# themattinthehatt/behavenet

Measured on AMD Instinct MI355X. Metric: AE training frames/sec (128x128x1, batch 256), higher is better.
Workload: dtype f32; 1 GPU; configs[1]: conv AE default arch, 1x128x128 f32 frames resident in HBM, 12 latents, batch 256 (chunks 200+56), fwd+bwd+Adam(amsgrad)

## Files before the change

behavenet_amd/_hip.py:

```python

import ctypes
import os

import torch

_LIB_NAME = 'libbehavenet_hip.so'
_LIB_PATH = os.environ.get('BN_HIP_LIB') or os.path.join(
    os.path.dirname(os.path.abspath(__file__)), _LIB_NAME)
_lib = None

ACT_NONE, ACT_LRELU, ACT_SIGMOID = 0, 1, 2

PROF_NONE, PROF_CONV_FWD, PROF_CONV_BWD_D, PROF_CONV_BWD_W = 0, 1, 2, 3
PROF_CONVT_FWD, PROF_CONVT_BWD_D, PROF_CONVT_BWD_W, PROF_ADAM = 4, 5, 6, 7
PROF_LINEAR_FWD, PROF_LINEAR_BWD = 8, 9

_c_int, _c_float, _c_size_t, _c_void_p = ctypes.c_int, ctypes.c_float, ctypes.c_size_t, ctypes.c_void_p

_CONV_GEOM = [_c_int] * 12
_ACT_WS = [_c_int, _c_float, _c_void_p, _c_size_t, _c_void_p]

OP_CONV_FWD, OP_CONV_BWD_D, OP_CONV_BWD_W = 1, 2, 3
OP_CONVT_FWD, OP_CONVT_BWD_D, OP_CONVT_BWD_W = 4, 5, 6

SIGNATURES = {
    'bn_version': (_c_int, []),
    'bn_build_arch': (ctypes.c_char_p, []),
    'bn_error_string': (ctypes.c_char_p, [_c_int]),
    'bn_set_force_generic': (_c_int, [_c_int]),
    'bn_set_bigk1_block_bytes': (_c_size_t, [_c_size_t]),
    'bn_conv_ws_bytes': (_c_size_t, [_c_int] + _CONV_GEOM),
    'bn_conv_taps_bytes': (_c_size_t, [_c_int] + _CONV_GEOM),
    'bn_conv_taps_pad': (_c_int, [_c_int, _c_void_p, _c_void_p, _c_void_p, _c_void_p]),
    'bn_conv_taps_hint': (_c_int, [_c_void_p, _c_void_p]),
    'bn_conv2d_fwd': (_c_int, [_c_void_p] * 4 + _CONV_GEOM + _ACT_WS),
    'bn_conv2d_fwd_u8_ws_bytes': (_c_size_t, _CONV_GEOM + [_c_int]),
    'bn_conv2d_fwd_u8': (_c_int, [_c_void_p] * 4 + _CONV_GEOM + _ACT_WS),
    'bn_conv2d_bwd_data': (_c_int, [_c_void_p] * 4 + _CONV_GEOM + _ACT_WS),
    'bn_conv2d_bwd_weight': (
        _c_int, [_c_void_p] * 4 + _CONV_GEOM + [_c_int, _c_void_p, _c_size_t, _c_void_p]),
    'bn_convT2d_fwd': (_c_int, [_c_void_p] * 4 + _CONV_GEOM + _ACT_WS),
    'bn_convT2d_bwd_data': (_c_int, [_c_void_p] * 4 + _CONV_GEOM + _ACT_WS),
    'bn_convT2d_bwd_weight': (
        _c_int, [_c_void_p] * 4 + _CONV_GEOM + [_c_int, _c_void_p, _c_size_t, _c_void_p]),
    'bn_batchnorm_ws_bytes': (_c_size_t, [_c_int, _c_int]),
    'bn_batchnorm_stats': (_c_int, [_c_void_p] * 3 + [_c_int] * 3 + [_c_void_p, _c_size_t, _c_void_p]),
    'bn_batchnorm_finalize': (_c_int, [_c_void_p] * 5 + [_c_int] + [_c_float] * 3 + [_c_void_p]),
    'bn_batchnorm_act_fwd': (_c_int, [_c_void_p] * 6 + [_c_int] * 4 + [_c_float, _c_void_p]),
    'bn_batchnorm_train_fwd_chunks': (
        _c_int, [_c_void_p] * 11 + [_c_int] * 3 + [_c_float, _c_int, _c_float, _c_void_p, _c_size_t,
                                                  _c_void_p]),
    'bn_batchnorm_act_bwd_chunks': (
        _c_int, [_c_void_p] * 10 + [_c_int, _c_void_p] + [_c_int] * 4 + [_c_float, _c_void_p, _c_size_t,
                                                                        _c_void_p]),
    'bn_batchnorm_act_bwd': (
        _c_int, [_c_void_p] * 9 + [_c_int] * 6 + [_c_float, _c_void_p, _c_size_t, _c_void_p]),
    'bn_batchnorm_moment': (_c_int, [_c_void_p] * 3 + [_c_int] * 3 + [_c_void_p, _c_size_t, _c_void_p]),
    'bn_batchnorm_bwd_reduce': (
        _c_int, [_c_void_p] * 7 + [_c_int] * 4 + [_c_float, _c_void_p, _c_size_t, _c_void_p]),
    'bn_batchnorm_bwd_apply': (
        _c_int, [_c_void_p] * 9 + [_c_int] * 3 + [_c_float, _c_int, _c_float, _c_void_p]),
    'bn_maxpool2d_fwd': (_c_int, [_c_void_p] * 3 + [_c_int] * 9 + [_c_void_p]),
    'bn_maxpool2d_bwd': (_c_int, [_c_void_p] * 3 + [_c_int] * 9 + [_c_void_p]),
    'bn_maxpool2d_act_fwd': (_c_int, [_c_void_p] * 3 + [_c_int] * 4 + [ctypes.c_float, _c_void_p]),
    'bn_conv2d_pool2_act_fwd': (_c_int, [_c_void_p] * 5 + _CONV_GEOM + [_c_int, _c_float, _c_void_p]),
    'bn_conv2d_pool2_act_ok': (_c_int, _CONV_GEOM),
    'bn_conv2d_pool2_bwd_weight_ws_bytes': (_c_size_t, _CONV_GEOM),
    'bn_conv2d_pool2_bwd_weight': (
        _c_int, [_c_void_p] * 6 + _CONV_GEOM + [_c_int, _c_float, _c_int, _c_void_p, _c_size_t, _c_void_p]),
    'bn_maxpool2d_act_bwd': (_c_int, [_c_void_p] * 4 + [_c_int] * 4 + [ctypes.c_float, _c_void_p]),
    'bn_maxunpool2d_fwd': (_c_int, [_c_void_p] * 3 + [_c_int] * 3 + [_c_void_p]),
    'bn_maxunpool2d_fwd_k2': (_c_int, [_c_void_p] * 3 + [_c_int] * 3 + [_c_void_p]),
    'bn_maxunpool2d_bwd': (_c_int, [_c_void_p] * 3 + [_c_int] * 3 + [_c_void_p]),
    'bn_act_fwd': (_c_int, [_c_void_p] * 2 + [_c_size_t, _c_int, _c_float, _c_void_p]),
    'bn_act_bwd': (_c_int, [_c_void_p] * 3 + [_c_size_t, _c_int, _c_float, _c_void_p]),
    'bn_linear_ws_bytes': (_c_size_t, [_c_int] * 3),
    'bn_linear_fwd': (_c_int, [_c_void_p] * 4 + [_c_int] * 3 + [_c_void_p, _c_size_t, _c_void_p]),
# ... 194 lines not shown
        _ptr(x, 'x'), _ptr(dy, 'dy'), _ptr(dw, 'dw'), _ptr(db, 'db', allow_none=True), *geom,
        int(accumulate), ws, nb, _stream()), 'bn_conv2d_bwd_weight')


def convT2d_fwd(x, w, b, geom, act, slope, w5=None):
    N, Ci, Hi, Wi, Co, R, S, st, ct, cl, Ho, Wo = geom
    y = torch.empty((N, Co, Ho, Wo), dtype=torch.float32, device=x.device)
    ws, nb = _workspace(OP_CONVT_FWD, geom, x.device)
    _taps_hint(w, w5)
    _check(load().bn_convT2d_fwd(
        _ptr(x, 'x'), _ptr(w, 'w'), _ptr(b, 'b', allow_none=True), _ptr(y, 'y'), *geom,
        act, slope, ws, nb, _stream()), 'bn_convT2d_fwd')
    return y


def convT2d_bwd_data(dy, w, geom, dact_src, dact, slope, w5=None):
    N, Ci, Hi, Wi = geom[:4]
    dx = torch.empty((N, Ci, Hi, Wi), dtype=torch.float32, device=dy.device)
    ws, nb = _workspace(OP_CONVT_BWD_D, geom, dy.device)
    _taps_hint(w, w5)
    _check(load().bn_convT2d_bwd_data(
        _ptr(dy, 'dy'), _ptr(w, 'w'), _ptr(dx, 'dx'), _ptr(dact_src, 'dact_src', allow_none=True),
        *geom, dact, slope, ws, nb, _stream()), 'bn_convT2d_bwd_data')
    return dx


def convT2d_bwd_weight(x, dy, dw, db, geom, accumulate):
    ws, nb = _workspace(OP_CONVT_BWD_W, geom, x.device)
    _check(lib_call('bn_convT2d_bwd_weight')(
        _ptr(x, 'x'), _ptr(dy, 'dy'), _ptr(dw, 'dw'), _ptr(db, 'db', allow_none=True), *geom,
        int(accumulate), ws, nb, _stream()), 'bn_convT2d_bwd_weight')


def set_force_generic(on):
    global _generic_epoch
    _generic_epoch += 1
    return bool(load().bn_set_force_generic(1 if on else 0))


def set_bigk1_block_bytes(nbytes):
    return int(load().bn_set_bigk1_block_bytes(int(nbytes)))


def lib_call(name):
    return getattr(load(), name)


def _bn_ws(n, c, device):
    nbytes = load().bn_batchnorm_ws_bytes(n, c)
    return _arena(device, nbytes, 'bn'), nbytes


def batchnorm_train_fwd(x, gamma, beta, running_mean, running_var, momentum, eps, act, slope, y=None):
    n, c = x.shape[0], x.shape[1]
    hw = x.numel() // (n * c)
    mean = torch.empty((c,), dtype=torch.float32, device=x.device)
    var = torch.empty_like(mean)
    invstd = torch.empty_like(mean)
    ws, nb = _bn_ws(n, c, x.device)
    _check(load().bn_batchnorm_stats(_ptr(x, 'x'), _ptr(mean, 'mean'), _ptr(var, 'var'), n, c, hw,
                                     ws, nb, _stream()), 'bn_batchnorm_stats')
    cnt = n * hw
    unbias = cnt / (cnt - 1.0) if cnt > 1 else 1.0
    _check(load().bn_batchnorm_finalize(
        _ptr(mean, 'mean'), _ptr(var, 'var'), _ptr(invstd, 'invstd'),
        _ptr(running_mean, 'running_mean', allow_none=True),
# ... 500 lines not shown
```

behavenet_amd/csrc/bn_fast.h:

```cpp
#pragma once
#include "bn_common.h"

struct BnFastPlan {
    bool supported;
    const char* kernel_name;
    size_t ws_bytes;
    int variant;
    int a, b, c, d;
};

BnFastPlan bn_fast_down_plan(const BnGeom& g);
BnFastPlan bn_fast_up_plan(const BnGeom& g);
BnFastPlan bn_fast_wgrad_plan(const BnGeom& g);

int bn_launch_down_fast(const BnFastPlan& plan, const float* big, const float* w,
                        const float* bias, float* out, const float* dact_src, const BnGeom& g,
                        int act, int dact, float slope, void* ws, hipStream_t st);
int bn_launch_up_fast(const BnFastPlan& plan, const float* small, const float* w,
                      const float* bias, float* out, const float* dact_src, const BnGeom& g,
                      int act, int dact, float slope, void* ws, hipStream_t st);
int bn_launch_wgrad_fast(const BnFastPlan& plan, const float* small, const float* big, float* dw,
                         const BnGeom& g, int accumulate, void* ws, hipStream_t st,
                         float* db = nullptr, int bias_side = 0, bool* bias_done = nullptr);

// ... 14 lines not shown
int bn_launch_down2(int MR, int NR, const float* big, const float* w, const float* bias,
                    float* out, const float* dact_src, const BnGeom& g, int act, int dact,
                    float slope, hipStream_t st, int splits = 1, void* ws = nullptr);

BnFastPlan bn_wgrad4_plan(const BnGeom& g);
int bn_launch_wgrad4(const BnFastPlan& plan, const float* small, const float* big, float* dw,
                     const BnGeom& g, int accumulate, void* ws, hipStream_t st, float* db,
                     int bias_side, bool* bias_done);

BnFastPlan bn_s5_up_plan(const BnGeom& g);
BnFastPlan bn_s5_wgrad_plan(const BnGeom& g);
int bn_launch_up_s5(const float* small, const float* w, const float* bias, float* out,
                    const float* dact_src, const BnGeom& g, int act, int dact, float slope,
                    hipStream_t st);
int bn_launch_wgrad_s5(const float* small, const float* big, float* dw, const BnGeom& g,
                       int accumulate, hipStream_t st);

BnFastPlan bn_edge_wgrad_plan(const BnGeom& g);
int bn_launch_edge_wgrad(const BnFastPlan& plan, const float* small, const float* big, float* dw,
                         const BnGeom& g, int accumulate, void* ws, hipStream_t st,
                         float* db = nullptr, int bias_side = 0, bool* bias_done = nullptr);
bool bn_s1c1_ok(const BnGeom& g);
int bn_launch_s1c1(const float* big, const float* w, const float* bias, float* out, const float* dact_src,
                   const BnGeom& g, int act, int dact, float slope, hipStream_t st);
bool bn_s1in1_ok(const BnGeom& g);
int bn_launch_s1in1(const float* big, const float* w, const float* bias, float* out, const float* dact_src,
                    const BnGeom& g, int act, int dact, float slope, hipStream_t st);
BnFastPlan bn_edge_down_plan(const BnGeom& g);
const char* bn_edge_down_kernel_name(const BnGeom& g, int act, bool has_dact, bool u8);
const char* bn_edge_up_kernel_name(const BnGeom& g, bool loss);
int bn_launch_edge_down(const float* big, const float* w, const float* bias, float* out,
                        const float* dact_src, const BnGeom& g, int act, int dact, float slope,
                        hipStream_t st, const unsigned char* u8 = nullptr);
BnFastPlan bn_edge_up_plan(const BnGeom& g);
int bn_launch_edge_up(const float* small, const float* w, const float* bias, float* out,
                      const BnGeom& g, int act, float slope, hipStream_t st,
                      const float* target = nullptr, const float* mask = nullptr,
                      float* dpre = nullptr, float* partial = nullptr);
int bn_edge_up_parts_per_frame(const BnGeom& g);

bool bn_qgemm_supported(const BnGeom& g);
size_t bn_qgemm_ws_bytes(int role, const BnGeom& g);
int bn_launch_qgemm_down(const float* big, const float* w, const float* bias, float* out,
                         const float* dact_src, const BnGeom& g, int act, int dact, float slope,
                         void* ws, hipStream_t st);
int bn_launch_qgemm_up(const float* small, const float* w, const float* bias, float* out,
                       const float* dact_src, const BnGeom& g, int act, int dact, float slope,
                       void* ws, hipStream_t st);
int bn_launch_qgemm_wgrad(const float* small, const float* big, float* dw, const BnGeom& g,
                          int accumulate, void* ws, hipStream_t st);

bool bn_qg2_up_supported(const BnGeom& g, int act, int dact);
int bn_launch_qg2_up(const float* small, const float* w, const float* bias, float* out,
                     const float* dact_src, const BnGeom& g, int act, int dact, float slope,
                     hipStream_t st);
bool bn_qg2_wgrad_supported(const BnGeom& g);
int bn_launch_qg2_wgrad(const float* small, const float* big, float* dw, const BnGeom& g,
                        int accumulate, float* db, int bias_side, hipStream_t st);

bool bn_s5win_supported(const BnGeom& g);
size_t bn_s5win_ws_bytes(int role, const BnGeom& g);
int bn_launch_s5win_down(const float* big, const float* w, const float* bias, float* out,
                         const float* dact_src, const BnGeom& g, int act, int dact, float slope,
                         void* ws, hipStream_t st);
int bn_launch_s5win_up(const float* small, const float* w, const float* bias, float* out,
                       const float* dact_src, const BnGeom& g, int act, int dact, float slope,
// ... 8 lines not shown
```

behavenet_amd/csrc/capi.hip:

```cpp
#include <math.h>
#include <stdio.h>
#include <stdlib.h>
#include <string.h>
#include <hip/hip_ext.h>
#include "bn_common.h"
#include "bn_launch.h"
#include "bn_fast.h"

namespace {
struct ProfState {
    int family = BN_PROF_NONE;
    int C = 0, K = 0;
    static const int kMaxSlots = 2048;
    hipEvent_t ev[4 * kMaxSlots];
    bool taken[kMaxSlots], bracketed[kMaxSlots];
    int created = 0;
    int used = 0;
    double total_ms = 0.0, main_ms = 0.0;
    long launches = 0, main_launches = 0;
    bool bracket = true;
    int nth = -1, seen = 0;
    char kernel_name[96] = "";
} g_prof;

// ... 1261 lines not shown
}

extern "C" int bn_convT2d_bwd_data(const float* dy, const float* w, float* dx,
                                   const float* dact_src, int N, int Ci, int Hi, int Wi, int Co,
                                   int R, int S, int stride, int crop_t, int crop_l, int Ho,
                                   int Wo, int dact, float slope, void* ws, size_t ws_bytes,
                                   bn_stream_t stream) {
    TapsHintDrop hint_drop;
    if (!dy || !w || !dx) return BN_E_BADARG;
    const BnGeom g = convT_geom(N, Ci, Hi, Wi, Co, R, S, stride, crop_t, crop_l, Ho, Wo);
    if (!bn_geom_ok(g)) return BN_E_BADARG;
    return run_down(BN_PROF_CONVT_BWD_D, dy, w, nullptr, dx, dact_src, g, BN_ACT_NONE, dact, slope,
                    ws, ws_bytes, (hipStream_t)stream);
}

extern "C" int bn_convT2d_bwd_weight(const float* x, const float* dy, float* dw, float* db, int N,
                                     int Ci, int Hi, int Wi, int Co, int R, int S, int stride,
                                     int crop_t, int crop_l, int Ho, int Wo, int accumulate,
                                     void* ws, size_t ws_bytes, bn_stream_t stream) {
    TapsHintDrop hint_drop;
    if (!x || !dy || !dw) return BN_E_BADARG;
    const BnGeom g = convT_geom(N, Ci, Hi, Wi, Co, R, S, stride, crop_t, crop_l, Ho, Wo);
    if (!bn_geom_ok(g)) return BN_E_BADARG;
    hipStream_t st = (hipStream_t)stream;
    bool bias_done = false;
    int rc = run_wgrad(BN_PROF_CONVT_BWD_W, x, dy, dw, g, accumulate, ws, ws_bytes, st, db, 2,
                       &bias_done);
    if (rc) return rc;
    if (db && !bias_done)
        rc = bn_launch_channel_sum(dy, db, N, Co, Ho * Wo, accumulate, ws, ws_bytes, st);
    return rc;
}

extern "C" int bn_act_fwd(const float* x, float* y, size_t n, int act, float slope,
                          bn_stream_t stream) {
    if (!x || !y || n == 0) return BN_E_BADARG;
    return bn_launch_act_fwd(x, y, n, act, slope, (hipStream_t)stream);
}

extern "C" int bn_act_bwd(const float* dy, const float* y, float* dpre, size_t n, int act,
                          float slope, bn_stream_t stream) {
    if (!dy || !y || !dpre) return BN_E_BADARG;
    if (n == 0) return 0;
    return bn_launch_act_bwd(dy, y, dpre, n, act, slope, (hipStream_t)stream);
}

extern "C" size_t bn_batchnorm_ws_bytes(int N, int C) {
    return (N > 0 && C > 0) ? bn_batchnorm_ws_bytes_impl(N, C) : 0;
}

extern "C" int bn_batchnorm_stats(const float* x, float* mean, float* var, int N, int C, int HW,
                                  void* ws, size_t ws_bytes, bn_stream_t stream) {
    if (!x || !mean || !var || N <= 0 || C <= 0 || HW <= 0) return BN_E_BADARG;
    if (!ws || ws_bytes < bn_batchnorm_ws_bytes_impl(N, C)) return BN_E_WORKSPACE;
    return bn_launch_bn_stats(x, mean, var, N, C, HW, ws, (hipStream_t)stream);
}

extern "C" int bn_batchnorm_finalize(const float* mean, const float* var, float* invstd,
                                     float* running_mean, float* running_var, int C, float eps,
                                     float momentum, float unbias, bn_stream_t stream) {
    if (!mean || !var || !invstd || C <= 0) return BN_E_BADARG;
    return bn_launch_bn_finalize(mean, var, invstd, running_mean, running_var, C, eps, momentum,
                                 unbias, (hipStream_t)stream);
}

extern "C" int bn_batchnorm_act_fwd(const float* x, const float* mean, const float* invstd,
// ... 313 lines not shown
```

behavenet_amd/csrc/conv_edge.hip:

```cpp
#include <hip/hip_ext.h>
#include <stdlib.h>
#include "bn_common.h"
#include "bn_fast.h"
#include "bn_reduce.h"

typedef float floatx16 __attribute__((ext_vector_type(16)));

#define ED_THREADS 256
#define ED_OOB 0x7fffffff

__device__ __forceinline__ float ed_ld(__amdgpu_buffer_rsrc_t r, int byte_off) {
    return __builtin_bit_cast(float, __builtin_amdgcn_raw_buffer_load_b32(r, byte_off, 0, 0));
}

#define WC_ROWS 4
#define WC_W 64
#define WC_TPX (WC_ROWS * WC_W)
#define WC_SP (WC_TPX + 2)
#define WC_IH (2 * WC_ROWS + 3)
#define WC_RW (2 * WC_W + 4)
#define WC_KS (32 * WC_TPX / ED_THREADS)

#define WC_DECODE_GRID()                                                                    \
    int bch, bx, G;                                                                         \
// ... 1433 lines not shown
                : launch_down_c1s<BN_ACT_NONE, false, true, 4>(u8, w, bias, out, nullptr, g, slope, st, e0, e1);
        return act == BN_ACT_LRELU
            ? launch_down_c1s<BN_ACT_LRELU, false, true, 2>(u8, w, bias, out, nullptr, g, slope, st, e0, e1)
            : launch_down_c1s<BN_ACT_NONE, false, true, 2>(u8, w, bias, out, nullptr, g, slope, st, e0, e1);
    }
    if (!dact_src && down_c1p_ok(g))
        return act == BN_ACT_LRELU
            ? launch_down_c1p<BN_ACT_LRELU>(big, w, bias, out, g, slope, st, e0, e1)
            : launch_down_c1p<BN_ACT_NONE>(big, w, bias, out, g, slope, st, e0, e1);
    if (dact_src || (g.CsS > 0 && g.CsS != g.Cs)) {
        if (act == BN_ACT_LRELU && !dact_src)
            return launch_down_c1s<BN_ACT_LRELU, false, false, 2>(big, w, bias, out, nullptr, g, slope, st, e0, e1);
        if (!dact_src)
            return launch_down_c1s<BN_ACT_NONE, false, false, 2>(big, w, bias, out, nullptr, g, slope, st, e0, e1);
        return launch_down_c1s<BN_ACT_NONE, true, false, 2>(big, w, bias, out, dact_src, g, slope, st, e0, e1);
    }
    if (down_c1w_ok(g))
        return act == BN_ACT_LRELU
            ? launch_down_c1w<BN_ACT_LRELU>(big, w, bias, out, g, slope, st, e0, e1)
            : launch_down_c1w<BN_ACT_NONE>(big, w, bias, out, g, slope, st, e0, e1);
    const int units = g.N * (g.Hs / DC_ROWS);
    const dim3 grid(down_c1_grid(units));
    if (act == BN_ACT_LRELU) {
        hipExtLaunchKernelGGL((k_down_c1<BN_ACT_LRELU, false>), grid, dim3(64), 0, st, e0, e1, 0,
                              big, w, bias, out, dact_src, g, slope, units);
    } else {
        hipExtLaunchKernelGGL((k_down_c1<BN_ACT_NONE, false>), grid, dim3(64), 0, st, e0, e1, 0,
                              big, w, bias, out, dact_src, g, slope, units);
    }
    BN_LAUNCH_CHECK();
    return 0;
}

#define UV_W 64

__device__ __forceinline__ float uv_shift_from_left(float v) {
    return __builtin_bit_cast(float, __builtin_amdgcn_mov_dpp(
        __builtin_bit_cast(int, v), 0x138 , 0xf, 0xf, true));
}
__device__ __forceinline__ float uv_shift_from_right(float v) {
    return __builtin_bit_cast(float, __builtin_amdgcn_mov_dpp(
        __builtin_bit_cast(int, v), 0x130 , 0xf, 0xf, true));
}

template <int R, bool LOSS, bool GENW = false>
__global__ __launch_bounds__(64) void k_up_c1v(
    const float* __restrict__ small, const float* __restrict__ w, const float* __restrict__ bias,
    float* __restrict__ out, const float* __restrict__ target, const float* __restrict__ mask,
    float* __restrict__ dpre, float* __restrict__ partial, BnGeom g, int act, float slope,
    int units) {
    constexpr int NR = R + 2;
    const int lane = threadIdx.x;
    const int strips = GENW ? (g.Hs + R - 1) / R : g.Hs / R;
    const int ncb = GENW ? (g.Ws + 61) / 62 : 1;
    const __amdgpu_buffer_rsrc_t rs = __builtin_amdgcn_make_buffer_rsrc(
        (void*)small, 0, (int)((size_t)g.N * g.Cs * g.Hs * g.Ws * 4), 0x00020000);
    const __amdgpu_buffer_rsrc_t rw = __builtin_amdgcn_make_buffer_rsrc(
        (void*)w, 0, (int)((size_t)g.Cs * g.Cb * 25 * 4), 0x00020000);

    static_assert((NR & 1) == 0, "input rows are kept as register pairs");
    struct Chan { floatx2p xx[NR / 2]; float wl; };

#pragma unroll 1
    for (int u = blockIdx.x; u < units; u += gridDim.x) {
        const int cbk = GENW ? u % ncb : 0;
        const int us = GENW ? u / ncb : u;
// ... 882 lines not shown
```

behavenet_amd/hip_functions.py:

```python

import collections.abc
import os

import torch

from behavenet_amd import _hip

LRELU_SLOPE = 0.05

_direct_grads = False


class accumulate_into_param_grads(object):

    def __enter__(self):
        global _direct_grads
        self._prev = _direct_grads
        _direct_grads = True

    def __exit__(self, *exc):
        global _direct_grads
        _direct_grads = self._prev
        return False

# ... 362 lines not shown
            else:
                h = _fwd(layer, h, params[2 * i].detach(), params[2 * i + 1].detach(),
                         w5=taps[i] if taps else None)
            acts.append(h)
        if _sign_tap is not None:
            rec = _sign_tap.setdefault(id(plan), [[] for _ in plan])
            for i, layer in enumerate(plan):
                if layer.act == _hip.ACT_LRELU:
                    rec[i].append((acts[i + 1] > 0).cpu())
        ctx.plan = plan
        ctx.taps = taps
        ctx.need_dx = x.requires_grad
        ctx.param_refs = params
        _note_use(params, any(ctx.needs_input_grad[3:]))
        ctx.save_for_backward(*acts, *params[0::2])
        return h

    @staticmethod
    def backward(ctx, dout):
        plan = ctx.plan
        dout = dout.contiguous()
        top = plan[-1]
        if top.act != _hip.ACT_NONE:
            dpre = _hip.act_bwd(dout, ctx.saved_tensors[len(plan)], top.act, LRELU_SLOPE)
        else:
            dpre = dout
        dx, grads = _stack_backward(ctx, dpre, first_param=3)
        return (None, dx, None) + tuple(grads)


_DGRAD_FIRST = os.environ.get('BN_DGRAD_FIRST', '0') == '1'


def _stack_backward(ctx, dpre, first_param):
    plan = ctx.plan
    n_layers = len(plan)
    saved = ctx.saved_tensors
    acts, weights = saved[:n_layers + 1], saved[n_layers + 1:2 * n_layers + 1]
    n = dpre.shape[0]
    grads = [None] * (2 * n_layers)
    taps = getattr(ctx, 'taps', None)
    tail = []
    for i in range(n_layers - 1, -1, -1):
        layer = plan[i]
        g = layer.geom(n)
        w = weights[i]
        x_in = acts[i]
        if x_in.dtype == torch.uint8:
            x_in = _hip.u8_to_unit_float(x_in) \
                if ctx.needs_input_grad[first_param + 2 * i] else None
        need_w = ctx.needs_input_grad[first_param + 2 * i]
        need_b = ctx.needs_input_grad[first_param + 1 + 2 * i]
        dpre_below = None
        if i > 0 and min(plan[i - 1].cin, plan[i - 1].cout) <= 4 and _DGRAD_FIRST:
            dact_src, dact = acts[i], plan[i - 1].act
            bwd_data = _hip.conv2d_bwd_data if layer.kind == 'conv' else _hip.convT2d_bwd_data
            dpre_below = bwd_data(dpre, w, g, dact_src, dact, LRELU_SLOPE, w5=taps[i] if taps else None)
        if need_w:
            gw = _grad_buffer(ctx.param_refs[2 * i])
            gb = _grad_buffer(ctx.param_refs[2 * i + 1]) if need_b else None
            direct = gw is not None and (gb is not None or not need_b)
            if direct:
                dw, db = gw, gb
            else:
                dw = torch.empty_like(w)
                db = torch.empty((layer.cout,), dtype=w.dtype, device=w.device) if need_b \
                    else None
            wgrad = _hip.conv2d_bwd_weight if layer.kind == 'conv' else _hip.convT2d_bwd_weight
            side = _side_stream(w.device) if (direct and _use_side_stream) else None
            if side is not None and not ctx.need_dx and i < _tail_on_main:
                tail.append(((wgrad, x_in, dpre, dw, db, g), ctx.param_refs[2 * i:2 * i + 2]))
            elif side is not None:
                main = torch.cuda.current_stream(w.device)
                ev = torch.cuda.Event()
                ev.record(main)
                with torch.cuda.stream(side):
                    side.wait_event(ev)
                    wgrad(x_in, dpre, dw, db, g, True)
                dpre.record_stream(side)
                x_in.record_stream(side)
                _report_ready(ctx.param_refs[2 * i:2 * i + 2])
            else:
                wgrad(x_in, dpre, dw, db, g, direct)
                if direct:
                    _report_ready(ctx.param_refs[2 * i:2 * i + 2])
            if not direct:
                grads[2 * i], grads[2 * i + 1] = dw, db
        if dpre_below is not None:
            dpre = dpre_below
        elif i > 0 or ctx.need_dx:
            dact_src = acts[i] if i > 0 else None
            dact = plan[i - 1].act if i > 0 else _hip.ACT_NONE
            w5 = taps[i] if taps else None
            if layer.kind == 'conv':
                dpre = _hip.conv2d_bwd_data(dpre, w, g, dact_src, dact, LRELU_SLOPE, w5=w5)
            else:
                dpre = _hip.convT2d_bwd_data(dpre, w, g, dact_src, dact, LRELU_SLOPE, w5=w5)
    for (wgrad, x_in, dy, dw, db, g), refs in tail:
        wgrad(x_in, dy, dw, db, g, True)
        _report_ready(refs)
    return (dpre if ctx.need_dx else None), grads


def conv_stack(plan, x, params, h1=None):
    return ConvStackFn.apply(plan, x, h1, *params)


_frame_scale_cache = {}


def _frame_scales(n, bounds, scales, device):
    key = (torch.device(device), int(n), tuple(bounds), tuple(float(s) for s in scales))
    hit = _frame_scale_cache.get(key)
    if hit is None:
        fs = torch.zeros(n, dtype=torch.float32)
        ci = torch.zeros(n, dtype=torch.int32)
        for c, ((beg, end), sc) in enumerate(zip(bounds, scales)):
            fs[beg:end] = float(sc)
            ci[beg:end] = c
        hit = (fs.to(device), ci.to(device))
        if len(_frame_scale_cache) > 64:
            _frame_scale_cache.clear()
        _frame_scale_cache[key] = hit
    return hit


class ConvStackSqErrFn(torch.autograd.Function):

    @staticmethod
    def forward(ctx, plan, x, target, mask, bounds, scales, want_xhat, *params):
        if plan[-1].kind != 'convT':
            raise ValueError('the fused pixel loss follows a transposed convolution')
        x = x.contiguous()
        target = target.contiguous()
        mask = mask.contiguous() if mask is not None else None
        acts = [x]
# ... 5 lines not shown
        top = plan[-1]
        n = h.shape[0]
        xhat, dpre, part = _hip.convT2d_fwd_sqerr(
            h, params[-2].detach(), params[-1].detach(), target, mask, top.geom(n), top.act,
            LRELU_SLOPE, bool(want_xhat))
        if _sign_tap is not None:
            rec = _sign_tap.setdefault(id(plan), [[] for _ in plan])
            for i, layer in enumerate(plan[:-1]):
                if layer.act == _hip.ACT_LRELU:
                    rec[i].append((acts[i + 1] > 0).cpu())
        out = torch.empty((len(bounds),), dtype=torch.float32, device=x.device)
        for c, ((beg, end), sc) in enumerate(zip(bounds, scales)):
            _hip.reduce_sum(part[beg:end], float(sc), out=out[c:c + 1])
        ctx.plan = plan
        ctx.taps = taps
        ctx.need_dx = x.requires_grad
        ctx.param_refs = params
        ctx.bounds, ctx.scales = list(bounds), [float(sc) for sc in scales]
        ctx.consumed = False
        _note_use(params, any(ctx.needs_input_grad[7:]))
        ctx.save_for_backward(*acts, dpre, *params[0::2])
        if xhat is not None:
            ctx.mark_non_differentiable(xhat)
        return out, xhat

    @staticmethod
    def backward(ctx, g, _g_xhat):
        if ctx.consumed:
            raise RuntimeError('ConvStackSqErrFn: backward twice (dL/dpre is scaled in place)')
        ctx.consumed = True
        n_layers = len(ctx.plan)
        dpre = ctx.saved_tensors[n_layers]
        fs, ci = _frame_scales(dpre.shape[0], ctx.bounds, ctx.scales, dpre.device)
        _hip.scale_frames(dpre, fs, g.contiguous(), ci)
        dx, grads = _stack_backward(ctx, dpre, first_param=7)
        return (None, dx, None, None, None, None, None) + tuple(grads)


def conv_stack_sq_err(plan, x, params, target, mask, bounds, scales, want_xhat=False):
    return ConvStackSqErrFn.apply(plan, x, target, mask, tuple(bounds), tuple(scales),
                                  bool(want_xhat), *params)


class FusedPixelLoss(object):

    def __init__(self, x_hat, chunk_terms, kind, bounds):
        self.x_hat = x_hat
        self.chunk_terms = chunk_terms
        self.kind = kind
        self.bounds = list(bounds)


_DEVICE_CONSTANTS = {}


def device_constant(values, device):
    key = (tuple(float(v) for v in values), str(device))
    t = _DEVICE_CONSTANTS.get(key)
    if t is None:
        if len(_DEVICE_CONSTANTS) > 256:
            _DEVICE_CONSTANTS.clear()
        t = torch.tensor(key[0], dtype=torch.float32, device=device)
        _DEVICE_CONSTANTS[key] = t
    return t


def pixel_loss_scales(kind, bounds, per_frame, chunk_sizes=None):
    sizes = chunk_sizes if chunk_sizes is not None else [end - beg for beg, end in bounds]
# ... 736 lines not shown
```

include/behavenet_hip.h:

```cpp
#ifndef BEHAVENET_HIP_H
#define BEHAVENET_HIP_H

#include <stddef.h>

#ifdef __cplusplus
extern "C" {
#endif

#define BN_E_BADARG   (-1)
#define BN_E_SHAPE    (-2)
#define BN_E_WORKSPACE (-3)

#define BN_ACT_NONE    0
#define BN_ACT_LRELU   1
#define BN_ACT_SIGMOID 2

typedef void* bn_stream_t;

int         bn_version(void);
const char* bn_build_arch(void);
const char* bn_error_string(int code);

#define BN_OP_CONV_FWD    1
#define BN_OP_CONV_BWD_D  2
// ... 9 lines not shown
                          int off_t, int off_l, int P, int Q);
int bn_conv_taps_pad(int n, const float* const* w, float* const* w5, const int* geoms, bn_stream_t stream);
int bn_conv_taps_hint(const float* w, const float* w5);

int bn_conv2d_fwd(const float* x, const float* w, const float* b, float* y,
                  int N, int C, int H, int W, int K, int R, int S, int stride,
                  int pad_t, int pad_l, int P, int Q,
                  int act, float slope, void* ws, size_t ws_bytes, bn_stream_t stream);

int bn_conv2d_bwd_data(const float* dy, const float* w, float* dx, const float* dact_src,
                       int N, int C, int H, int W, int K, int R, int S, int stride,
                       int pad_t, int pad_l, int P, int Q,
                       int dact, float slope, void* ws, size_t ws_bytes, bn_stream_t stream);

int bn_conv2d_bwd_weight(const float* x, const float* dy, float* dw, float* db,
                         int N, int C, int H, int W, int K, int R, int S, int stride,
                         int pad_t, int pad_l, int P, int Q,
                         int accumulate, void* ws, size_t ws_bytes, bn_stream_t stream);

int bn_convT2d_fwd(const float* x, const float* w, const float* b, float* y,
                   int N, int Ci, int Hi, int Wi, int Co, int R, int S, int stride,
                   int crop_t, int crop_l, int Ho, int Wo,
                   int act, float slope, void* ws, size_t ws_bytes, bn_stream_t stream);

int bn_convT2d_bwd_data(const float* dy, const float* w, float* dx, const float* dact_src,
                        int N, int Ci, int Hi, int Wi, int Co, int R, int S, int stride,
                        int crop_t, int crop_l, int Ho, int Wo,
                        int dact, float slope, void* ws, size_t ws_bytes, bn_stream_t stream);

int bn_convT2d_bwd_weight(const float* x, const float* dy, float* dw, float* db,
                          int N, int Ci, int Hi, int Wi, int Co, int R, int S, int stride,
                          int crop_t, int crop_l, int Ho, int Wo,
                          int accumulate, void* ws, size_t ws_bytes, bn_stream_t stream);

int bn_act_fwd(const float* x, float* y, size_t n, int act, float slope, bn_stream_t stream);
int bn_act_bwd(const float* dy, const float* y, float* dpre, size_t n,
               int act, float slope, bn_stream_t stream);

int bn_maxpool2d_fwd(const float* x, float* y, int* idx, int planes, int H, int W, int Ho, int Wo,
                     int k, int stride, int pad_t, int pad_l, bn_stream_t stream);
int bn_maxpool2d_bwd(const float* dy, const int* idx, float* dx, int planes, int H, int W,
                     int Ho, int Wo, int k, int stride, int pad_t, int pad_l, bn_stream_t stream);
int bn_conv2d_pool2_act_fwd(const float* x, const float* w, const float* b, float* y, int* idx,
                            int N, int C, int H, int W, int K, int R, int S, int stride,
                            int pad_t, int pad_l, int P, int Q, int act, float slope, bn_stream_t stream);
int bn_conv2d_pool2_act_ok(int N, int C, int H, int W, int K, int R, int S, int stride,
                           int pad_t, int pad_l, int P, int Q);
size_t bn_conv2d_pool2_bwd_weight_ws_bytes(int N, int C, int H, int W, int K, int R, int S, int stride,
                                           int pad_t, int pad_l, int P, int Q);
int bn_conv2d_pool2_bwd_weight(const float* x, const float* dy, const float* y, const int* idx, float* dw, float* db,
                               int N, int C, int H, int W, int K, int R, int S, int stride,
                               int pad_t, int pad_l, int P, int Q, int act, float slope, int accumulate,
                               void* ws, size_t ws_bytes, bn_stream_t stream);
int bn_maxpool2d_act_fwd(const float* x, float* y, int* idx, int planes, int H, int W, int act, float slope,
                         bn_stream_t stream);
int bn_maxpool2d_act_bwd(const float* dy, const float* y, const int* idx, float* dx, int planes, int H, int W,
                         int act, float slope, bn_stream_t stream);
int bn_maxunpool2d_fwd(const float* x, const int* idx, float* y, int planes, int in_plane,
                       int out_plane, bn_stream_t stream);
int bn_maxunpool2d_fwd_k2(const float* x, const int* idx, float* y, int planes, int Hi, int Wi, bn_stream_t stream);
int bn_maxunpool2d_bwd(const float* dy, const int* idx, float* dx, int planes, int in_plane,
                       int out_plane, bn_stream_t stream);

size_t bn_batchnorm_ws_bytes(int N, int C);
int bn_batchnorm_stats(const float* x, float* mean, float* var, int N, int C, int HW,
                       void* ws, size_t ws_bytes, bn_stream_t stream);
// ... 127 lines not shown
```

Measured before the change: 58890 frames/s.

## Fuse loss scaling, dgrad and wgrad for final transposed-conv layer backward

Adds a single kernel for the last convT layer (1 output channel, 5x5 stride 2) that applies the per-frame loss scales to the output gradient on the fly. In the same pass it computes the data gradient with the LeakyReLU derivative applied and accumulates the weight and bias gradients from one double-buffered LDS staging of the small and big tensors. This replaces a separate scale_frames pass plus separate bwd-data and bwd-weight kernels, each of which reread the full-resolution gradient. A small partial-sum reduction kernel finishes dw and db, and the path falls back when the shape is unsupported.

```diff
diff --git a/behavenet_amd/_hip.py b/behavenet_amd/_hip.py
--- a/behavenet_amd/_hip.py
+++ b/behavenet_amd/_hip.py
@@ -43,6 +43,10 @@
     'bn_convT2d_bwd_data': (_c_int, [_c_void_p] * 4 + _CONV_GEOM + _ACT_WS),
     'bn_convT2d_bwd_weight': (
         _c_int, [_c_void_p] * 4 + _CONV_GEOM + [_c_int, _c_void_p, _c_size_t, _c_void_p]),
+    'bn_convT2d_bwd_fused_ws_bytes': (_c_size_t, _CONV_GEOM + [_c_int]),
+    'bn_convT2d_bwd_fused': (
+        _c_int, [_c_void_p] * 6 + _CONV_GEOM + [_c_void_p] * 3 +
+        [_c_int, _c_float, _c_int, _c_void_p, _c_size_t, _c_void_p]),
     'bn_batchnorm_ws_bytes': (_c_size_t, [_c_int, _c_int]),
     'bn_batchnorm_stats': (_c_int, [_c_void_p] * 3 + [_c_int] * 3 + [_c_void_p, _c_size_t, _c_void_p]),
     'bn_batchnorm_finalize': (_c_int, [_c_void_p] * 5 + [_c_int] + [_c_float] * 3 + [_c_void_p]),
@@ -303,6 +307,37 @@
         int(accumulate), ws, nb, _stream()), 'bn_convT2d_bwd_weight')
 
 
+E_SHAPE = -2
+_fused_bytes = {}
+
+
+def convT2d_bwd_fused_ws_bytes(geom, dact):
+    key = (_generic_epoch, int(dact)) + tuple(geom)
+    v = _fused_bytes.get(key)
+    if v is None:
+        v = _fused_bytes[key] = int(load().bn_convT2d_bwd_fused_ws_bytes(*geom, int(dact)))
+    return v
+
+
+def convT2d_bwd_fused(x, dy, w, dw, db, geom, frame_scale, group_scale, group_of_frame, dact, slope, accumulate):
+    nb = convT2d_bwd_fused_ws_bytes(geom, dact)
+    if nb == 0:
+        return None
+    N, Ci, Hi, Wi = geom[:4]
+    dx = torch.empty((N, Ci, Hi, Wi), dtype=torch.float32, device=dy.device)
+    ws = _arena(dy.device, nb)
+    rc = load().bn_convT2d_bwd_fused(
+        _ptr(x, 'x'), _ptr(dy, 'dy'), _ptr(w, 'w'), _ptr(dx, 'dx'), _ptr(dw, 'dw'),
+        _ptr(db, 'db', allow_none=True), *geom, _ptr(frame_scale, 'frame_scale'),
+        _ptr(group_scale, 'group_scale', allow_none=True),
+        _ptr(group_of_frame, 'group_of_frame', dtype=torch.int32, allow_none=True),
+        int(dact), slope, int(accumulate), ws, nb, _stream())
+    if rc == E_SHAPE:
+        return None
+    _check(rc, 'bn_convT2d_bwd_fused')
+    return dx
+
+
 def set_force_generic(on):
     global _generic_epoch
     _generic_epoch += 1
diff --git a/behavenet_amd/csrc/bn_fast.h b/behavenet_amd/csrc/bn_fast.h
--- a/behavenet_amd/csrc/bn_fast.h
+++ b/behavenet_amd/csrc/bn_fast.h
@@ -70,6 +70,12 @@
 int bn_launch_edge_down(const float* big, const float* w, const float* bias, float* out,
                         const float* dact_src, const BnGeom& g, int act, int dact, float slope,
                         hipStream_t st, const unsigned char* u8 = nullptr);
+bool bn_edge_bwd_fused_ok(const BnGeom& g);
+size_t bn_edge_bwd_fused_ws_bytes(const BnGeom& g);
+int bn_launch_edge_bwd_fused(const float* small, const float* big, const float* w, float* out, float* dw,
+                             float* db, const float* frame_scale, const float* group_scale,
+                             const int* group_of_frame, const BnGeom& g, float slope, int accumulate, void* ws,
+                             hipStream_t st);
 BnFastPlan bn_edge_up_plan(const BnGeom& g);
 int bn_launch_edge_up(const float* small, const float* w, const float* bias, float* out,
                       const BnGeom& g, int act, float slope, hipStream_t st,
diff --git a/behavenet_amd/csrc/capi.hip b/behavenet_amd/csrc/capi.hip
--- a/behavenet_amd/csrc/capi.hip
+++ b/behavenet_amd/csrc/capi.hip
@@ -1317,6 +1317,34 @@
     return rc;
 }
 
+static bool convT_bwd_fused_served(const BnGeom& g, int dact) {
+    return bn_geom_ok(g) && !force_generic() && dact == BN_ACT_LRELU && bn_edge_bwd_fused_ok(g);
+}
+
+extern "C" size_t bn_convT2d_bwd_fused_ws_bytes(int N, int Ci, int Hi, int Wi, int Co, int R, int S, int stride,
+                                                int crop_t, int crop_l, int Ho, int Wo, int dact) {
+    const BnGeom g = convT_geom(N, Ci, Hi, Wi, Co, R, S, stride, crop_t, crop_l, Ho, Wo);
+    return convT_bwd_fused_served(g, dact) ? bn_edge_bwd_fused_ws_bytes(g) : 0;
+}
+
+extern "C" int bn_convT2d_bwd_fused(const float* x, const float* dy, const float* w, float* dx, float* dw,
+                                    float* db, int N, int Ci, int Hi, int Wi, int Co, int R, int S, int stride,
+                                    int crop_t, int crop_l, int Ho, int Wo, const float* frame_scale,
+                                    const float* group_scale, const int* group_of_frame, int dact, float slope,
+                                    int accumulate, void* ws, size_t ws_bytes, bn_stream_t stream) {
+    TapsHintDrop hint_drop;
+    if (!x || !dy || !w || !dx || !dw || !frame_scale) return BN_E_BADARG;
+    if ((group_scale == nullptr) != (group_of_frame == nullptr)) return BN_E_BADARG;
+    const BnGeom g = convT_geom(N, Ci, Hi, Wi, Co, R, S, stride, crop_t, crop_l, Ho, Wo);
+    if (!bn_geom_ok(g)) return BN_E_BADARG;
+    if (!convT_bwd_fused_served(g, dact) || !aligned16_all(x, dy, dx)) return BN_E_SHAPE;
+    if (!ws || ws_bytes < bn_edge_bwd_fused_ws_bytes(g)) return BN_E_WORKSPACE;
+    hipStream_t st = (hipStream_t)stream;
+    BnProfScope prof(BN_PROF_CONVT_BWD_D, g.Cb, g.Cs, "k_bwd_c1f", st);
+    return bn_launch_edge_bwd_fused(x, dy, w, dx, dw, db, frame_scale, group_scale, group_of_frame, g, slope,
+                                    accumulate, ws, st);
+}
+
 extern "C" int bn_act_fwd(const float* x, float* y, size_t n, int act, float slope,
                           bn_stream_t stream) {
     if (!x || !y || n == 0) return BN_E_BADARG;
diff --git a/behavenet_amd/csrc/conv_edge.hip b/behavenet_amd/csrc/conv_edge.hip
--- a/behavenet_amd/csrc/conv_edge.hip
+++ b/behavenet_amd/csrc/conv_edge.hip
@@ -1489,6 +1489,307 @@
     return 0;
 }
 
+#define WF_SCALES 128
+#define WF_LDS ((2 * WD_BUF + WF_SCALES) * 4)
+
+__global__ __launch_bounds__(ED_THREADS, 2) void k_bwd_c1f(
+    const float* __restrict__ small, const float* __restrict__ big, const float* __restrict__ w,
+    float* __restrict__ out, float* __restrict__ part, float* __restrict__ bias_part,
+    const float* __restrict__ frame_scale, const float* __restrict__ group_scale,
+    const int* __restrict__ group_of_frame, BnGeom g, float slope, int n_stages, int stages_per_frame) {
+    extern __shared__ __attribute__((aligned(16))) float wsm[];
+    const int tid = threadIdx.x, lane = tid & 63;
+    const int wv = __builtin_amdgcn_readfirstlane(tid >> 6);
+    const int li = lane & 31, kk = lane >> 5;
+    const int PQ = g.Hs * g.Ws, HWb = g.Hb * g.Wb;
+    const int bx = blockIdx.x, G = gridDim.x;
+
+    const __amdgpu_buffer_rsrc_t rs = __builtin_amdgcn_make_buffer_rsrc(
+        (void*)small, 0, (int)((size_t)g.N * g.Cs * PQ * 4), 0x00020000);
+    const __amdgpu_buffer_rsrc_t rb = __builtin_amdgcn_make_buffer_rsrc(
+        (void*)(big - g.Wb), 0, (int)(((size_t)g.N * HWb + g.Wb) * 4), 0x00020000);
+    const __amdgpu_buffer_rsrc_t ro = __builtin_amdgcn_make_buffer_rsrc(
+        (void*)out, 0, (int)((size_t)g.N * g.Cs * PQ * 4), 0x00020000);
+
+    float wd[13];
+#pragma unroll
+    for (int t = 0; t < 13; ++t) {
+        const int tap = 2 * t + kk;
+        wd[t] = (tap < 25 && li < g.Cs) ? w[li * 25 + tap] : 0.f;
+    }
+    for (int e = tid; e < 2 * WD_BUF; e += ED_THREADS) {
+        const int wo = e % WD_BUF;
+        if (wo < 32 * WD_SP && wo / WD_SP >= g.Cs) wsm[e] = 0.f;
+    }
+    const int svo = (wv * PQ + 4 * lane) * 4;
+    int bvo[2], bcls = 0;
+#pragma unroll
+    for (int k = 0; k < 2; ++k) {
+        const int e = lane + 64 * (wv + 4 * k);
+        const int y = e / (WD_RW / 4), c = e - y * (WD_RW / 4);
+        const bool ok = e < WD_BG && c >= 1 && c <= 2 * WC_W / 4;
+        bvo[k] = ok ? (y * g.Wb + 4 * (c - 1)) * 4 : ED_OOB;
+        bcls |= ((y == 0 ? 1 : 0) | (y >= WC_IH - 2 ? 2 : 0)) << (2 * k);
+    }
+    auto issue_dma = [&](const int d, const int buf, const int st) __attribute__((always_inline)) {
+        const int n = st / stages_per_frame;
+        const int p0 = (st - n * stages_per_frame) * WC_ROWS;
+        float* img = wsm + buf * WD_BUF;
+        if (d < 8) {
+            if (wv + 4 * d < g.Cs)
+                wd_dma16(rs, img + (wv + 4 * d) * WD_SP, svo, ((n * g.Cs + 4 * d) * g.Hs + p0) * g.Ws * 4);
+        } else {
+            const int k = d - 8;
+            if (64 * (wv + 4 * k) < WD_BGP) {
+                const int smask = ((p0 == 0 ? 1 : 0) | (p0 + WC_ROWS >= g.Hs ? 2 : 0)) << (2 * k);
+                wd_dma16(rb, img + 32 * WD_SP + 4 * 64 * (wv + 4 * k), (bcls & smask) ? ED_OOB : bvo[k],
+                         (n * g.Hb + 2 * p0) * g.Wb * 4);
+            }
+        }
+    };
+    if (tid < WF_SCALES && bx + tid * G < n_stages) {
+        const int n = (bx + tid * G) / stages_per_frame;
+        float s = frame_scale[n];
+        if (group_scale) s *= group_scale[group_of_frame[n]];
+        wsm[2 * WD_BUF + tid] = s;
+    }
+
+    floatx16 acc[2];
+#pragma unroll
+    for (int h = 0; h < 2; ++h)
+#pragma unroll
+        for (int e = 0; e < 16; ++e) acc[h][e] = 0.f;
+    float bsum = 0.f;
+
+    const int tap = li < 25 ? li : 0;
+    const int tr = tap / 5, ts = tap - tr * 5;
+    const int aq0 = (li * WD_SP + wv * WC_W + kk) * 4;
+    const int bq0 = (32 * WD_SP + (2 * wv + tr) * WD_RW + ts + 2 * kk + 3) * 4;
+    const int gq0 = (32 * WD_SP + 2 * wv * WD_RW + 2 * li + 3) * 4;
+    const int gqA0 = gq0 + kk * 4, gqB0 = gq0 + kk * (WD_RW - 4) * 4;
+    const int hq0 = (4 * kk * WD_SP + wv * WC_W + li) * 4;
+    const int dq0 = (32 * WD_SP + (1 + (tid >> 5)) * WD_RW + 4 + 4 * (tid & 31)) * 4;
+    const int st_lane = (4 * kk * PQ + li) * 4;
+    const char* sm = reinterpret_cast<const char*>(wsm);
+
+    int st = bx;
+    if (st < n_stages) {
+#pragma unroll
+        for (int d = 0; d < 10; ++d) issue_dma(d, 0, st);
+    }
+    asm volatile("s_waitcnt vmcnt(0)" ::: "memory");
+    int cur = 0, ks = 0;
+    for (; st < n_stages; st += G) {
+        asm volatile("s_waitcnt vmcnt(32)" ::: "memory");
+        __syncthreads();
+        const int nx = st + G;
+        const bool more = nx < n_stages;
+        const float sc = wsm[2 * WD_BUF + ks];
+        const int bo = cur * (WD_BUF * 4);
+        const int n = st / stages_per_frame;
+        const int p0 = (st - n * stages_per_frame) * WC_ROWS;
+
+        const int aq = bo + aq0, bq = bo + bq0;
+        const int gqA = bo + gqA0, gqB = bo + gqB0;
+        const int hq = bo + hq0;
+        auto load_w = [&](const int c, float (&A)[8], float (&B)[8]) __attribute__((always_inline)) {
+#pragma unroll
+            for (int j = 0; j < 8; ++j) {
+                A[j] = *reinterpret_cast<const float*>(sm + aq + 8 * (8 * c + j));
+                B[j] = *reinterpret_cast<const float*>(sm + bq + 16 * (8 * c + j));
+            }
+        };
+        auto mul_w = [&](const int c, const float (&A)[8], const float (&B)[8]) __attribute__((always_inline)) {
+#pragma unroll
+            for (int j = 0; j < 8; ++j) {
+                const int t = 8 * c + j;
+                acc[t & 1] = __builtin_amdgcn_mfma_f32_32x32x2f32(A[j], B[j] * sc, acc[t & 1], 0, 0, 0);
+                if (t >= 2 && t < 12) { if (more) issue_dma(t - 2, cur ^ 1, nx); }
+            }
+        };
+        auto load_g = [&](const int T0, const int T1, float (&B)[14]) __attribute__((always_inline)) {
+#pragma unroll
+            for (int t = T0; t < T1; ++t) {
+                const int t0 = (((2 * t) / 5) * WD_RW + (2 * t) % 5) * 4;
+                const int gq = ((2 * t) % 5 == 4 && t != 12) ? gqB : gqA;
+#pragma unroll
+                for (int qh = 0; qh < 2; ++qh)
+                    B[2 * (t - T0) + qh] = *reinterpret_cast<const float*>(sm + gq + t0 + 256 * qh);
+            }
+        };
+        floatx16 dacc[2];
+        auto mul_g = [&](const int T0, const int T1, const float (&B)[14]) __attribute__((always_inline)) {
+#pragma unroll
+            for (int t = T0; t < T1; ++t)
+#pragma unroll
+                for (int qh = 0; qh < 2; ++qh)
+                    dacc[qh] = __builtin_amdgcn_mfma_f32_32x32x2f32(wd[t], B[2 * (t - T0) + qh] * sc, dacc[qh], 0, 0, 0);
+        };
+        auto load_h = [&](const int qh, float (&d)[16]) __attribute__((always_inline)) {
+#pragma unroll
+            for (int e = 0; e < 16; ++e) {
+                const int chb = (e & 3) + 8 * (e >> 2);
+                d[e] = *reinterpret_cast<const float*>(sm + hq + (chb * WD_SP + 32 * qh) * 4);
+            }
+        };
+        const int row_off = (n * g.Cs * g.Hs + (p0 + wv)) * WC_W * 4;
+        auto store_h = [&](const int qh, const float (&d)[16]) __attribute__((always_inline)) {
+#pragma unroll
+            for (int e = 0; e < 16; ++e) {
+                const int chb = (e & 3) + 8 * (e >> 2);
+                const bool ok = chb + 4 * kk < g.Cs;
+                float v = dacc[qh][e];
+                v *= d[e] > 0.f ? 1.f : slope;
+                __builtin_amdgcn_raw_buffer_store_b32(__builtin_bit_cast(int, v), ro, ok ? st_lane : ED_OOB,
+                                                      row_off + (chb * PQ + 32 * qh) * 4, 0);
+            }
+        };
+#define WF_FENCE() __builtin_amdgcn_sched_barrier(0)
+        float wa0[8], wb0[8], wa1[8], wb1[8], gb0[14], gb1[14], hd0[16], hd1[16];
+        load_w(0, wa0, wb0);
+        WF_FENCE();
+        load_w(1, wa1, wb1);
+        WF_FENCE();
+        mul_w(0, wa0, wb0);
+        WF_FENCE();
+        load_w(2, wa0, wb0);
+        WF_FENCE();
+        mul_w(1, wa1, wb1);
+        WF_FENCE();
+        load_w(3, wa1, wb1);
+        WF_FENCE();
+        mul_w(2, wa0, wb0);
+        WF_FENCE();
+        load_g(0, 7, gb0);
+        {
+            typedef float wf_f4 __attribute__((ext_vector_type(4)));
+            const wf_f4 v = *reinterpret_cast<const wf_f4*>(sm + bo + dq0);
+            bsum += sc * ((v.x + v.y) + (v.z + v.w));
+        }
+        WF_FENCE();
+        mul_w(3, wa1, wb1);
+        WF_FENCE();
+        load_g(7, 13, gb1);
+#pragma unroll
+        for (int qh = 0; qh < 2; ++qh)
+#pragma unroll
+            for (int e = 0; e < 16; ++e) dacc[qh][e] = 0.f;
+        WF_FENCE();
+        mul_g(0, 7, gb0);
+        WF_FENCE();
+        load_h(0, hd0);
+        WF_FENCE();
+        mul_g(7, 13, gb1);
+        WF_FENCE();
+        load_h(1, hd1);
+        WF_FENCE();
+        store_h(0, hd0);
+        store_h(1, hd1);
+#undef WF_FENCE
+        cur ^= 1;
+        ++ks;
+    }
+
+    __syncthreads();
+    float* red = wsm;
+#pragma unroll
+    for (int e = 0; e < 16; ++e) red[(wv * 16 + e) * 64 + lane] = acc[0][e] + acc[1][e];
+    red[4096 + tid] = bsum;
+    __syncthreads();
+    if (wv == 0) {
+        if (li < 25) {
+#pragma unroll
+            for (int e = 0; e < 16; ++e) {
+                const float v = (red[e * 64 + lane] + red[(16 + e) * 64 + lane]) +
+                                (red[(32 + e) * 64 + lane] + red[(48 + e) * 64 + lane]);
+                const int a = (e & 3) + 8 * (e >> 2) + 4 * kk;
+                if (a < g.Cs) part[(size_t)bx * (g.Cs * 25) + a * 25 + li] = v;
+            }
+        }
+        if (bias_part) {
+            float s = (red[4096 + lane] + red[4160 + lane]) + (red[4224 + lane] + red[4288 + lane]);
+#pragma unroll
+            for (int m = 32; m >= 1; m >>= 1) s += __shfl_xor(s, m, 64);
+            if (lane == 0) bias_part[bx] = s;
+        }
+    }
+}
+
+__global__ __launch_bounds__(1024) void k_sum_partials_wb(
+    const float* __restrict__ part_a, float* __restrict__ out_a, int total_a, const float* __restrict__ part_b,
+    float* __restrict__ out_b, int total_b, int splits, int accumulate, int blocks_a) {
+    __shared__ float red[16][64];
+    const bool job_b = (int)blockIdx.x >= blocks_a;
+    const float* part = job_b ? part_b : part_a;
+    float* out = job_b ? out_b : out_a;
+    const int total = job_b ? total_b : total_a;
+    const int il = threadIdx.x & 63, zl = threadIdx.x >> 6;
+    const int nz = blockDim.x >> 6;
+    const int i = ((int)blockIdx.x - (job_b ? blocks_a : 0)) * 64 + il;
+    float s0 = 0.f, s1 = 0.f, s2 = 0.f, s3 = 0.f;
+    if (i < total) {
+        int z = zl;
+        for (; z + 3 * nz < splits; z += 4 * nz) {
+            s0 += part[(size_t)z * total + i];
+            s1 += part[(size_t)(z + nz) * total + i];
+            s2 += part[(size_t)(z + 2 * nz) * total + i];
+            s3 += part[(size_t)(z + 3 * nz) * total + i];
+        }
+        for (; z < splits; z += nz) s0 += part[(size_t)z * total + i];
+    }
+    red[zl][il] = (s0 + s1) + (s2 + s3);
+    __syncthreads();
+    if (nz == 16 && zl < 4)
+        red[zl][il] = (red[zl][il] + red[zl + 4][il]) + (red[zl + 8][il] + red[zl + 12][il]);
+    if (nz == 16) __syncthreads();
+    if (zl == 0 && i < total) {
+        const float v = (red[0][il] + red[1][il]) + (red[2][il] + red[3][il]);
+        out[i] = accumulate ? out[i] + v : v;
+    }
+}
+
+bool bn_edge_bwd_fused_ok(const BnGeom& g) {
+    if (g.R != 5 || g.S != 5 || g.stride != 2 || g.Cb != 1 || g.Cs > 32 || g.CsS != 0 || g.KV != 0 || g.K0 != 0)
+        return false;
+    if (g.pt != 1 || g.pl != 1) return false;
+    if (g.Ws != WC_W || (g.Hs % WC_ROWS) != 0 || g.Hb != 2 * g.Hs || g.Wb != 2 * g.Ws) return false;
+    if ((size_t)g.N * g.Cs * g.Hs * g.Ws * 4 >= 0x7fff0000ull) return false;
+    if ((size_t)g.N * g.Cb * g.Hb * g.Wb * 4 >= 0x7fff0000ull) return false;
+    return true;
+}
+
+size_t bn_edge_bwd_fused_ws_bytes(const BnGeom& g) {
+    const int G = wgrad_c1_grid(g);
+    return ((size_t)G * g.Cs * 25 + (size_t)G) * sizeof(float);
+}
+
+int bn_launch_edge_bwd_fused(const float* small, const float* big, const float* w, float* out, float* dw,
+                             float* db, const float* frame_scale, const float* group_scale,
+                             const int* group_of_frame, const BnGeom& g, float slope, int accumulate, void* ws,
+                             hipStream_t st) {
+    if (!bn_edge_bwd_fused_ok(g)) return BN_E_SHAPE;
+    static bool attr_set = false;
+    if (!attr_set) {
+        hipError_t e = hipFuncSetAttribute((const void*)k_bwd_c1f, hipFuncAttributeMaxDynamicSharedMemorySize, WF_LDS);
+        if (e != hipSuccess) return (int)e;
+        attr_set = true;
+    }
+    const int spf = g.Hs / WC_ROWS, n_stages = g.N * spf;
+    const int G = wgrad_c1_grid(g);
+    if ((n_stages + G - 1) / G > WF_SCALES) return BN_E_SHAPE;
+    float* part = (float*)ws;
+    float* bias_part = db ? part + (size_t)G * g.Cs * 25 : nullptr;
+    BN_LAUNCH_MAIN(k_bwd_c1f, dim3(G), dim3(ED_THREADS), WF_LDS, st, small, big, w, out, part, bias_part,
+                   frame_scale, group_scale, group_of_frame, g, slope, n_stages, spf);
+    BN_LAUNCH_CHECK();
+    const int total = g.Cs * 25, blocks_a = (total + 63) / 64;
+    const int threads = (G >= 128 && total <= 16384) ? 1024 : 256;
+    hipLaunchKernelGGL(k_sum_partials_wb, dim3(blocks_a + (db ? 1 : 0)), dim3(threads), 0, st, (const float*)part, dw,
+                       total, (const float*)bias_part, db, 1, G, accumulate, blocks_a);
+    BN_LAUNCH_CHECK();
+    return 0;
+}
+
 #define UV_W 64
 
 __device__ __forceinline__ float uv_shift_from_left(float v) {
diff --git a/behavenet_amd/hip_functions.py b/behavenet_amd/hip_functions.py
--- a/behavenet_amd/hip_functions.py
+++ b/behavenet_amd/hip_functions.py
@@ -418,7 +418,7 @@
 _DGRAD_FIRST = os.environ.get('BN_DGRAD_FIRST', '0') == '1'
 
 
-def _stack_backward(ctx, dpre, first_param):
+def _stack_backward(ctx, dpre, first_param, top_scales=None):
     plan = ctx.plan
     n_layers = len(plan)
     saved = ctx.saved_tensors
@@ -427,7 +427,14 @@
     grads = [None] * (2 * n_layers)
     taps = getattr(ctx, 'taps', None)
     tail = []
-    for i in range(n_layers - 1, -1, -1):
+    top_done = False
+    if top_scales is not None:
+        dh = _top_fused(ctx, dpre, first_param, top_scales, acts, weights, grads)
+        if dh is None:
+            _hip.scale_frames(dpre, *top_scales)
+        else:
+            dpre, top_done = dh, True
+    for i in range(n_layers - 1 - int(top_done), -1, -1):
         layer = plan[i]
         g = layer.geom(n)
         w = weights[i]
@@ -488,6 +495,40 @@
     return (dpre if ctx.need_dx else None), grads
 
 
+_D4_FUSED = os.environ.get('BN_D4_FUSED', '1') != '0'
+
+
+def _top_fused(ctx, dpre, first_param, top_scales, acts, weights, grads):
+    plan = ctx.plan
+    i = len(plan) - 1
+    layer = plan[i]
+    if not _D4_FUSED or i == 0 or layer.kind != 'convT' or not ctx.needs_input_grad[first_param + 2 * i]:
+        return None
+    g = layer.geom(dpre.shape[0])
+    dact = plan[i - 1].act
+    if not _hip.convT2d_bwd_fused_ws_bytes(g, dact):
+        return None
+    w = weights[i]
+    need_b = ctx.needs_input_grad[first_param + 1 + 2 * i]
+    gw = _grad_buffer(ctx.param_refs[2 * i])
+    gb = _grad_buffer(ctx.param_refs[2 * i + 1]) if need_b else None
+    direct = gw is not None and (gb is not None or not need_b)
+    if direct:
+        dw, db = gw, gb
+    else:
+        dw = torch.empty_like(w)
+        db = torch.empty((layer.cout,), dtype=w.dtype, device=w.device) if need_b else None
+    fs, gs, ci = top_scales
+    dh = _hip.convT2d_bwd_fused(acts[i], dpre, w, dw, db, g, fs, gs, ci, dact, LRELU_SLOPE, direct)
+    if dh is None:
+        return None
+    if direct:
+        _report_ready(ctx.param_refs[2 * i:2 * i + 2])
+    else:
+        grads[2 * i], grads[2 * i + 1] = dw, db
+    return dh
+
+
 def conv_stack(plan, x, params, h1=None):
     return ConvStackFn.apply(plan, x, h1, *params)
 
@@ -559,8 +600,7 @@
         n_layers = len(ctx.plan)
         dpre = ctx.saved_tensors[n_layers]
         fs, ci = _frame_scales(dpre.shape[0], ctx.bounds, ctx.scales, dpre.device)
-        _hip.scale_frames(dpre, fs, g.contiguous(), ci)
-        dx, grads = _stack_backward(ctx, dpre, first_param=7)
+        dx, grads = _stack_backward(ctx, dpre, first_param=7, top_scales=(fs, g.contiguous(), ci))
         return (None, dx, None, None, None, None, None) + tuple(grads)
 
 
diff --git a/include/behavenet_hip.h b/include/behavenet_hip.h
--- a/include/behavenet_hip.h
+++ b/include/behavenet_hip.h
@@ -65,6 +65,14 @@
                           int N, int Ci, int Hi, int Wi, int Co, int R, int S, int stride,
                           int crop_t, int crop_l, int Ho, int Wo,
                           int accumulate, void* ws, size_t ws_bytes, bn_stream_t stream);
+
+size_t bn_convT2d_bwd_fused_ws_bytes(int N, int Ci, int Hi, int Wi, int Co, int R, int S, int stride,
+                                     int crop_t, int crop_l, int Ho, int Wo, int dact);
+int bn_convT2d_bwd_fused(const float* x, const float* dy, const float* w, float* dx, float* dw, float* db,
+                         int N, int Ci, int Hi, int Wi, int Co, int R, int S, int stride,
+                         int crop_t, int crop_l, int Ho, int Wo,
+                         const float* frame_scale, const float* group_scale, const int* group_of_frame,
+                         int dact, float slope, int accumulate, void* ws, size_t ws_bytes, bn_stream_t stream);
 
 int bn_act_fwd(const float* x, float* y, size_t n, int act, float slope, bn_stream_t stream);
 int bn_act_bwd(const float* dy, const float* y, float* dpre, size_t n,
```

Result: no change. 59470 frames/s (median of 6 runs) (+1.0%).
